# NLESC-JCER/Fortran_Davidson

Hardware: AMD Instinct MI355X
Metric: Davidson iterations/sec (dense DPR solve, matrix resident in HBM) + A*V HBM GB/s vs roofline (higher is better)
Workload: dtype f64

## Files before the change

fortran_davidson_amd/csrc/engine_apply.hip:

```cpp
#include "engine_internal.h"

bool inner_f32_tiles(E* e, OpDesc& o) {
  if (e->inner_bits != 32 || o.kind != DAV_KIND_DENSE || o.storage != 1 || o.a32_refused) return false;
  if (o.a32_valid) return true;
  const size_t count = (size_t)std::max<int64_t>(e->sym.ntiles, 1) * SYM_TB * SYM_TB;
  if (!o.a32 && pool_malloc(&o.a32, sizeof(float) * count) != hipSuccess) {
    (void)hipGetLastError();
    o.a32 = nullptr;
    o.a32_refused = true;
    return false;
  }
  launch_tiles_to_f32(e->stream, o.a, o.a32, (int64_t)count);
  o.a32_valid = true;
  return true;
}

static double* sym_slab_t(const E* e, const SymLaunch& L) { return e->sym_slab + (int64_t)L.ngroups * L.dstride; }
static void sym_sweep(E* e, const SymLaunch& L, const OpDesc& o, const SymSet& set, const double* xt) {
  if (L.nitems == 0) return;
  const SymPlan* pl = L.plan;
  const void* tiles = L.use32 ? (const void*)o.a32 : (const void*)o.a;
  double *slabD = e->sym_slab, *slabT = sym_slab_t(e, L);
  const int64_t xs = e->xt_group_stride, ds = L.dstride, ts = L.tstride;
  switch (L.family) {
    case SYM_ROW_STORED:
      return launch_matvec_sym(e->stream, o.a, set.row_off, set.items, set.nitems, xt, L.kk, slabD, slabT, L.ngroups, xs, ds, ts);
    case SYM_ROW_GENERATED:
      return launch_matvec_sym_generated(e->stream, op_params(o), e->n, set.items, set.nitems, xt, L.kk, slabD, slabT, L.ngroups, xs, ds, ts);
    case SYM_SUPER:
      return launch_matvec_sym9(e->stream, L.R, o.kind != DAV_KIND_DENSE, tiles, L.use32, set.row_off, o.kind != DAV_KIND_DENSE ? op_params(o) : OpParams{},
                                e->n, e->sym_nb, pl->items, pl->nitems, pl->zslot_begin, xt, L.kk, slabD, slabT, L.nwg, xs, ds, ts, e->tune.sym_mfma4 != 0);
    case SYM_WIDE:
    case SYM_WIDE_F32:
      return launch_matvec_symw(e->stream, L.nbw, L.tall, L.use32, tiles, set.row_off, e->sym_nb, pl->items, pl->nitems, pl->zslot_begin, xt, L.kk, slabD, slabT, L.nwg, xs, ds, ts);
    case SYM_WIDE_GENERATED:
      return launch_matvec_symw_generated(e->stream, op_params(o), e->n, e->sym_nb, pl->items, pl->nitems, pl->zslot_begin, xt, L.kk, slabD, slabT, L.nwg, xs, ds, ts);
  }
}

static void count_apply(E* e, int which, int kk) { if (which == DAV_OP_A) { e->st.applies += 1; e->st.apply_cols += kk; } }

static int pack_operand(E* e, const double* src, int kk, bool gather) {
  launch_pack_xt(e->stream, src, e->ldp, e->nloc, e->nslab, kk, e->xt, e->xt_group_stride, e->row0);
  if (!gather) return 0;
  const int ngroups = (kk + 15) / 16;
  CollGroup grp(e);
  CHK(grp.begin(5, 8.0 * (double)e->nslab * 16 * ngroups * e->nranks));
  for (int g = 0; g < ngroups; ++g)
    CHK(coll_allgather(e, e->xt + g * e->xt_group_stride + e->row0 * 16, e->xt + g * e->xt_group_stride, (size_t)e->nslab * 16));
  return grp.end("all-gather of the new block", e->stream);
}

static void sym_reduce_groups(E* e, const SymLaunch& L, const SymSet& set, const int64_t* owned, double* out, int64_t chunk_rows, bool accumulate) {
  const int64_t total_rows = (int64_t)e->nranks * e->nslab;
  const double* slabT = sym_slab_t(e, L);
  for (int g = 0; g < L.ngroups; ++g) {
    const int kg = std::min(16, L.kk - 16 * g);
    const double *d = e->sym_slab + g * L.dstride, *t = slabT + g * L.tstride;
    double* og = out + (size_t)g * 16 * (size_t)(chunk_rows ? total_rows : e->ldp);
    if (L.plan)
      launch_sym9_reduce(e->stream, d, t, L.plan->row_begin, L.plan->zslot_begin, owned, L.plan->next_owned, L.R, e->sym_nb, e->nloc, kg, og, e->ldp,
                         chunk_rows, total_rows, accumulate);
    else
      launch_sym_reduce(e->stream, d, t, set.row_begin, owned, e->sym_nb, e->nloc, kg, og, e->ldp, chunk_rows, total_rows, accumulate);
  }
}

static int ensure_sym_wpart(E* e) {
  if (e->sym_wpart) return 0;
  HIPCHK(pool_malloc(&e->sym_wpart, sizeof(double) * (size_t)e->nranks * (size_t)e->nslab * 64));
  HIPCHK(pool_malloc(&e->sym_wrecv, sizeof(double) * (size_t)e->nslab * 64));
  return 0;
}

static int sym_scatter_to_panel(E* e, int kk, double* dst, bool accumulate, const char* what, double* h0 = nullptr, size_t h0_count = 0) {
  const size_t wstride = (size_t)e->nranks * (size_t)e->nslab * 16, rstride = (size_t)e->nslab * 16;
  const int ngroups = (kk + 15) / 16;
  CollGroup grp(e);
  CHK(grp.begin(6, 8.0 * (double)e->nslab * kk * e->nranks));
  for (int g = 0; g < ngroups; ++g)
    CHK(coll_reduce_scatter(e, e->sym_wpart + g * wstride, e->sym_wrecv + g * rstride, (size_t)e->nslab * std::min(16, kk - 16 * g)));
  if (h0) CHK(coll_allreduce(e, h0, h0_count));
  CHK(grp.end(what, e->stream));
  for (int g = 0; g < ngroups; ++g)
    launch_chunk_to_panel(e->stream, e->sym_wrecv + g * rstride, e->nslab, e->nloc, e->nloc_pad, std::min(16, kk - 16 * g), dst + (int64_t)(16 * g) * e->ldp, e->ldp, accumulate);
  return 0;
}

static double sym_stored_bytes(const E* e, const OpDesc& o, const SymSet& set, bool partial, bool use32) {
  return o.kind != DAV_KIND_DENSE ? 0.0 : (use32 ? 4.0 : 8.0) * (partial ? (double)set.ntiles * SYM_TB * SYM_TB : 0.5 * (double)e->n * ((double)e->n + 1.0) / e->nranks);
}

static int apply_sym_overlapped(E* e, int which, OpDesc& o, const double* src, int k, double* dst, bool timed, bool inner) {
  const int step = 32;
  const int nchunks = (k + step - 1) / step;
  if (!e->ov_ready) {
    hipStream_t cs = nullptr;
    hipEvent_t evs[8] = {};
    double* bufs[4] = {};
    auto undo = [&]() {
      for (hipEvent_t v : evs) if (v) (void)hipEventDestroy(v);
      for (double* b : bufs) if (b) (void)pool_free(b);
      if (cs) (void)hipStreamDestroy(cs);
    };
    int prio_least = 0, prio_greatest = 0;
    if (hipDeviceGetStreamPriorityRange(&prio_least, &prio_greatest) != hipSuccess) { (void)hipGetLastError(); prio_greatest = 0; }
    bool ok = hipStreamCreateWithPriority(&cs, hipStreamNonBlocking, prio_greatest) == hipSuccess;
    for (int i = 0; ok && i < 8; ++i) ok = hipEventCreateWithFlags(&evs[i], hipEventDisableTiming) == hipSuccess;
    for (int i = 0; ok && i < 2; ++i) {
      ok = pool_malloc(&bufs[i], sizeof(double) * (size_t)e->nranks * (size_t)e->nslab * 32) == hipSuccess &&
           pool_malloc(&bufs[2 + i], sizeof(double) * (size_t)e->nslab * 32) == hipSuccess;
    }
    if (!ok) {
      (void)hipGetLastError();
      undo();
      return 2;
    }
    e->comm_stream = cs;
// ... 433 lines not shown
  }
  const bool sym = e->op[which].storage == 1;
  *bytes = (sym ? sym_stored_bytes(e, e->op[which], e->sym, false, false) : 8.0 * (double)e->nloc * (double)e->n) + 16.0 * (double)e->n * k;
  *flops = 2.0 * (sym ? (double)e->n / e->nranks : (double)e->nloc) * (double)e->n * k;
  e->st = saved;
  return 0;
}

extern "C" int dav_bench_stream3(dav_handle_t e, int64_t doubles, int reps, double* copy_GBps, double* triad_GBps, double* read_GBps) {
  CHK(bind(e));
  const int64_t n = doubles > 0 ? doubles / 2 * 2 : (int64_t)1 << 28;
  if (reps <= 0) reps = 5;
  double *a = nullptr, *b = nullptr, *c = nullptr;
  hipEvent_t ev[2] = {nullptr, nullptr};
  auto cleanup = [&]() {
    pool_free(a); pool_free(b); pool_free(c);
    for (hipEvent_t v : ev) if (v) hipEventDestroy(v);
  };
  if (pool_malloc(&a, sizeof(double) * n) != hipSuccess || pool_malloc(&b, sizeof(double) * n) != hipSuccess ||
      pool_malloc(&c, sizeof(double) * n) != hipSuccess || hipEventCreate(&ev[0]) != hipSuccess || hipEventCreate(&ev[1]) != hipSuccess) {
    (void)hipGetLastError();
    cleanup();
    return fail("dav_bench_stream: could not allocate three arrays of " + std::to_string(n) + " doubles");
  }
  double out[3] = {0.0, 0.0, 0.0};
  int rc = 0;
  auto run = [&]() -> int {
    HIPCHK(hipMemsetAsync(b, 0, sizeof(double) * n, e->stream));
    HIPCHK(hipMemsetAsync(c, 0, sizeof(double) * n, e->stream));
    for (int mode = 0; mode < 3; ++mode) {
      launch_stream(e->stream, mode, a, b, c, 0.5, n);
      HIPCHK(hipEventRecord(ev[0], e->stream));
      for (int r = 0; r < reps; ++r) launch_stream(e->stream, mode, a, b, c, 0.5, n);
      HIPCHK(hipEventRecord(ev[1], e->stream));
      HIPCHK(hipEventSynchronize(ev[1]));
      float ms = 0;
      HIPCHK(hipEventElapsedTime(&ms, ev[0], ev[1]));
      out[mode] = (mode == 1 ? 3.0 : 2.0) * 8.0 * (double)n * reps / (ms * 1e-3) / 1e9;
    }
    return 0;
  };
  rc = run();
  cleanup();
  if (rc != 0) return rc;
  if (copy_GBps) *copy_GBps = out[0];
  if (triad_GBps) *triad_GBps = out[1];
  if (read_GBps) *read_GBps = out[2];
  return 0;
}
extern "C" int dav_bench_stream(dav_handle_t e, int64_t doubles, int reps, double* copy_GBps, double* triad_GBps) {
  return dav_bench_stream3(e, doubles, reps, copy_GBps, triad_GBps, nullptr);
}

extern "C" int dav_bench_harness_rate(dav_handle_t e, int iters, double* entries_per_s) {
  CHK(bind(e));
  if (iters <= 0) iters = 2000;
  const int wgs = 512;
  double* out = nullptr;
  hipEvent_t ev[2] = {nullptr, nullptr};
  HIPCHK(pool_malloc(&out, sizeof(double) * (size_t)wgs * 512));
  auto cleanup = [&]() { pool_free(out); for (hipEvent_t v : ev) if (v) hipEventDestroy(v); };
  auto run = [&]() -> int {
    HIPCHK(hipEventCreate(&ev[0]));
    HIPCHK(hipEventCreate(&ev[1]));
    launch_harness_rate(e->stream, out, wgs, 200);
    HIPCHK(hipEventRecord(ev[0], e->stream));
    launch_harness_rate(e->stream, out, wgs, iters);
    HIPCHK(hipEventRecord(ev[1], e->stream));
    HIPCHK(hipEventSynchronize(ev[1]));
    float ms = 0;
    HIPCHK(hipEventElapsedTime(&ms, ev[0], ev[1]));
    *entries_per_s = (double)wgs * 512.0 * iters / (ms * 1e-3);
    return 0;
  };
  const int rc = run();
  cleanup();
  return rc;
}
```

fortran_davidson_amd/csrc/engine_internal.h:

```cpp
#pragma once
#include "davidson_hip_private.h"
#include "kernels.h"
#include "ingest.h"

#include <dlfcn.h>
#include <fcntl.h>
#include <pthread.h>
#include <sys/mman.h>
#include <sys/stat.h>
#include <unistd.h>
#include <rccl/rccl.h>

#include <algorithm>
#include <chrono>
#include <condition_variable>
#include <ctime>
#include <mutex>
#include <cmath>
#include <cstdio>
#include <cstring>
#include <numeric>
#include <string>
#include <thread>
#include <vector>

#pragma GCC visibility push(hidden)
extern thread_local std::string g_err;
int fail(const std::string& msg);
#define HIPCHK(call)                                                                                  \
  do {                                                                                                \
    hipError_t e_ = (call);                                                                           \
    if (e_ != hipSuccess) {                                                                           \
      (void)hipGetLastError();      \
      return fail(std::string(#call) + " failed: " + hipGetErrorString(e_) + " (" __FILE__ ":" +      \
                  std::to_string(__LINE__) + ")");                                                    \
    }                                                                                                 \
  } while (0)
#define CHK(call)            \
  do {                       \
    int r_ = (call);         \
    if (r_ != 0) return r_;  \
  } while (0)

hipError_t pool_malloc_raw(void** p, size_t bytes);
hipError_t pool_host_malloc_raw(void** p, size_t bytes, unsigned flags);
hipError_t pool_free(void* p);
hipError_t pool_host_free(void* p);
size_t pool_idle_device_bytes(int device);
void pool_begin_of_destroy();
void pool_end_of_destroy();
hipError_t pool_stream_get(hipStream_t* st);
void pool_stream_put(hipStream_t st, int device);
template <class T> inline hipError_t pool_malloc(T** p, size_t bytes) { return pool_malloc_raw((void**)p, bytes); }
template <class T> inline hipError_t pool_host_malloc(T** p, size_t bytes, unsigned flags) { return pool_host_malloc_raw((void**)p, bytes, flags); }


struct Rccl {
  void* lib = nullptr;
  ncclResult_t (*GetUniqueId)(ncclUniqueId*) = nullptr;
  ncclResult_t (*CommInitRank)(ncclComm_t*, int, ncclUniqueId, int) = nullptr;
  ncclResult_t (*CommDestroy)(ncclComm_t) = nullptr;
  ncclResult_t (*AllGather)(const void*, void*, size_t, ncclDataType_t, ncclComm_t, hipStream_t) = nullptr;
  ncclResult_t (*AllReduce)(const void*, void*, size_t, ncclDataType_t, ncclRedOp_t, ncclComm_t, hipStream_t) = nullptr;
  ncclResult_t (*Broadcast)(const void*, void*, size_t, ncclDataType_t, int, ncclComm_t, hipStream_t) = nullptr;
  ncclResult_t (*ReduceScatter)(const void*, void*, size_t, ncclDataType_t, ncclRedOp_t, ncclComm_t, hipStream_t) = nullptr;
  ncclResult_t (*Send)(const void*, size_t, ncclDataType_t, int, ncclComm_t, hipStream_t) = nullptr;
  ncclResult_t (*Recv)(void*, size_t, ncclDataType_t, int, ncclComm_t, hipStream_t) = nullptr;
  ncclResult_t (*GroupStart)() = nullptr;
  ncclResult_t (*GroupEnd)() = nullptr;
  const char* (*GetErrorString)(ncclResult_t) = nullptr;
  ncclResult_t (*CommCount)(const ncclComm_t, int*) = nullptr;
};
extern Rccl g_rccl;
int rccl_load();
#define NCCLCHK(call)                                                                              \
  do {                                                                                             \
    ncclResult_t r_ = (call);                                                                      \
// ... 350 lines not shown
```

fortran_davidson_amd/csrc/k_matvec_sym.hip:

```cpp
#include "kernels.h"
#include <cstdlib>
#include <type_traits>

__device__ __forceinline__ const double* sym_tile(const double* tiles, const int64_t* __restrict__ row_off, int I, int J) {
  return tiles + (row_off[I] + J) * (int64_t)(SYM_TB * SYM_TB);
}

constexpr int SYM8_DEPTH = 3;

template <bool GEN>
__global__ __launch_bounds__(512, 1) void matvec_sym8_kernel(const double* __restrict__ tiles, const int64_t* __restrict__ row_off,
                                                             const int* __restrict__ items,
                                                             const double* __restrict__ xt, double* __restrict__ slabD,
                                                             double* __restrict__ slabT, int kcols, int npair,
                                                             int64_t xt_gstride, int64_t slabD_gstride, int64_t slabT_gstride,
                                                             OpParams op, int64_t n) {
  int item, grp;
  if (npair == 2) {
    const int nfull = (int)(gridDim.x / 16) * 16;
    if ((int)blockIdx.x < nfull) {
      item = (blockIdx.x / 16) * 8 + (blockIdx.x % 8);
      grp = (blockIdx.x / 8) % 2;
    } else {
      item = nfull / 2 + (blockIdx.x - nfull) / 2;
// ... 163 lines not shown
#pragma unroll
          for (int reg = 0; reg < 4; ++reg) zs[4 * reg] = z[reg];
        }
      }
      if ((q & 3) == 3 && ((q >> 2) + 1) % zslots == 0) {
        __syncthreads();
        flush_tiles((q >> 2) + 1 - zslots, zslots);
        __syncthreads();
      }
    }
#pragma unroll
    for (int u = 0; u < 4; ++u) b[u] = bn[u];
  };
  int q = 0;
  for (; q < nq_off; ++q) unit(std::true_type{}, q);
  if ((nq_off >> 2) % zslots != 0) {
    __syncthreads();
    flush_tiles((nq_off >> 2) - (nq_off >> 2) % zslots, (nq_off >> 2) % zslots);
  }
  for (; q < nunits; ++q) unit(std::false_type{}, q);

  double* outD = slabD + (int64_t)items[4 * item + 3] * 16 * SYM_TB;
#pragma unroll
  for (int hs = 0; hs < 4; ++hs) {
    __syncthreads();
#pragma unroll
    for (int par = 0; par < 2; ++par)
#pragma unroll
      for (int reg = 0; reg < 4; ++reg) tw[c * RS + 2 * (g + 4 * reg) + par] = acc[hs][par][reg];
    __syncthreads();
#pragma unroll
    for (int t = 0; t < 2; ++t) {
      const int e = threadIdx.x + 512 * t;
      const int hh = e >> 9, bc = (e >> 5) & 15, r = e & 31;
      const double* rp = tr + (hh * 4) * TRW + bc * RS + r;
      if (bc < kcols) outD[(int64_t)bc * SYM_TB + 128 * hh + 32 * hs + r] = (rp[0] + rp[TRW]) + (rp[2 * TRW] + rp[3 * TRW]);
    }
  }
}

void launch_matvec_sym(hipStream_t st, const double* tiles, const int64_t* row_off, const int* items_dev, int nitems, const double* xt, int kcols,
                       double* slabD, double* slabT, int npair, int64_t xt_gstride, int64_t slabD_gstride, int64_t slabT_gstride) {
  hipLaunchKernelGGL(matvec_sym8_kernel<false>, dim3(nitems * npair), dim3(512), 0, st, tiles, row_off, items_dev, xt, slabD, slabT, kcols,
                     npair, xt_gstride, slabD_gstride, slabT_gstride, OpParams{}, (int64_t)0);
}
void launch_matvec_sym_generated(hipStream_t st, OpParams op, int64_t n, const int* items_dev, int nitems, const double* xt, int kcols,
                                 double* slabD, double* slabT, int npair, int64_t xt_gstride, int64_t slabD_gstride,
                                 int64_t slabT_gstride) {
  hipLaunchKernelGGL(matvec_sym8_kernel<true>, dim3(nitems * npair), dim3(512), 0, st, (const double*)nullptr, (const int64_t*)nullptr, items_dev, xt, slabD,
                     slabT, kcols, npair, xt_gstride, slabD_gstride, slabT_gstride, op, n);
}

__global__ __launch_bounds__(256) void sym_reduce_kernel(const double* __restrict__ slabD, const double* __restrict__ slabT,
                                                         const int* __restrict__ row_item_begin, const int64_t* __restrict__ owned,
                                                         int nb, int ncol16, int64_t nloc, int k, double* __restrict__ dst, int64_t ldd,
                                                         int64_t chunk_rows, int64_t total_rows, int accumulate) {
  const int J = blockIdx.x, col = blockIdx.y, r = threadIdx.x;
  if (col >= k) return;
  double sum = 0.0;
  for (int it = row_item_begin[J]; it < row_item_begin[J + 1]; ++it)
    sum += slabD[((int64_t)it * ncol16 + col) * SYM_TB + r];
  auto zt = [&](int I) { return (!owned || owned[I] >= 0) ? slabT[((((int64_t)I * (I - 1) / 2 + J) * ncol16) + col) * SYM_TB + r] : 0.0; };
  double s0 = 0.0, s1 = 0.0, s2 = 0.0, s3 = 0.0;
  int I = J + 1;
  for (; I + 3 < nb; I += 4) { s0 += zt(I); s1 += zt(I + 1); s2 += zt(I + 2); s3 += zt(I + 3); }
  for (; I < nb; ++I) s0 += zt(I);
  sum += (s0 + s1) + (s2 + s3);
  int64_t row = (int64_t)J * SYM_TB + r;
  if (chunk_rows > 0) {
    if (row < total_rows) dst[(row / chunk_rows) * (chunk_rows * k) + (int64_t)col * chunk_rows + row % chunk_rows] = sum;
  } else {
    dst[(int64_t)col * ldd + row] = row < nloc ? (accumulate ? dst[(int64_t)col * ldd + row] + sum : sum) : 0.0;
  }
}

void launch_sym_reduce(hipStream_t st, const double* slabD, const double* slabT, const int* row_item_begin_dev, const int64_t* owned,
                       int nb, int64_t nloc, int k, double* dst, int64_t ldd, int64_t chunk_rows, int64_t total_rows, bool accumulate) {
  hipLaunchKernelGGL(sym_reduce_kernel, dim3(nb, k), dim3(256), 0, st, slabD, slabT, row_item_begin_dev, owned, nb, 16, nloc, k,
                     dst, ldd, chunk_rows, total_rows, accumulate && chunk_rows == 0 ? 1 : 0);
}

__global__ __launch_bounds__(256) void generate_sym_tiles_kernel(double* __restrict__ row_tiles, int I, int64_t n, uint64_t seed,
                                                                 double sparsity, int use_diag, double diag_val) {
  const int64_t J = blockIdx.x;
  double* tile = row_tiles + J * (int64_t)(SYM_TB * SYM_TB);
  int64_t gi = (int64_t)I * SYM_TB + threadIdx.x;
  for (int cc = 0; cc < 16; ++cc) {
    int64_t lc = blockIdx.y * 16 + cc, gj = J * SYM_TB + lc;
    double v = 0.0;
    if (gi < n && gj < n) v = dav_hashed_entry(seed, sparsity, use_diag, diag_val, gi, gj);
    tile[lc * SYM_TB + threadIdx.x] = v;
  }
}

void launch_generate_sym_tiles(hipStream_t st, double* tiles, const int64_t* row_off_host, int nb, int64_t n, uint64_t seed,
                               double sparsity, int use_diag, double diag_val) {
  for (int I = 0; I < nb; ++I)
    if (row_off_host[I] >= 0)
      hipLaunchKernelGGL(generate_sym_tiles_kernel, dim3((unsigned)(I + 1), SYM_TB / 16), dim3(SYM_TB), 0, st,
                         tiles + row_off_host[I] * (int64_t)(SYM_TB * SYM_TB), I, n, seed, sparsity, use_diag, diag_val);
}

__device__ __forceinline__ double sym_entry(const double* tiles, const int64_t* __restrict__ row_off, int64_t i, int64_t j) {
  if (i < j) { int64_t t = i; i = j; j = t; }
  int I = (int)(i / SYM_TB), J = (int)(j / SYM_TB);
  if (row_off[I] < 0) return 0.0;
  return sym_tile(tiles, row_off, I, J)[(j % SYM_TB) * SYM_TB + (i % SYM_TB)];
}

__global__ void diag_sym_kernel(const double* __restrict__ tiles, const int64_t* __restrict__ row_off, int64_t n, int64_t nrows,
                                double* __restrict__ diag) {
  int64_t i = (int64_t)blockIdx.x * 256 + threadIdx.x;
  if (i < nrows) diag[i] = i < n ? sym_entry(tiles, row_off, i, i) : 0.0;
}
void launch_diag_sym(hipStream_t st, const double* tiles, const int64_t* row_off, int64_t n, int64_t nrows, double* diag) {
  hipLaunchKernelGGL(diag_sym_kernel, dim3((unsigned)((nrows + 255) / 256)), dim3(256), 0, st, tiles, row_off, n, nrows, diag);
}

__global__ void gather_columns_sym_kernel(const double* __restrict__ tiles, const int64_t* __restrict__ row_off, int64_t n,
                                          int64_t nrows_pad, const int64_t* __restrict__ idx, double* __restrict__ dst, int64_t ldd) {
  int64_t i = (int64_t)blockIdx.x * 256 + threadIdx.x;
  int c = blockIdx.y;
  if (i < nrows_pad) dst[(int64_t)c * ldd + i] = i < n ? sym_entry(tiles, row_off, i, idx[c]) : 0.0;
}
void launch_gather_columns_sym(hipStream_t st, const double* tiles, const int64_t* row_off, int64_t n, int64_t nrows_pad,
                               const int64_t* idx_dev, int k, double* dst, int64_t ldd) {
  hipLaunchKernelGGL(gather_columns_sym_kernel, dim3((unsigned)((nrows_pad + 255) / 256), k), dim3(256), 0, st, tiles, row_off, n,
                     nrows_pad, idx_dev, dst, ldd);
}

__global__ void gather_columns_sym_rs_kernel(const double* __restrict__ tiles, const int64_t* __restrict__ row_off, int64_t n,
// ... 36 lines not shown
```

fortran_davidson_amd/csrc/k_matvec_sym9.hip:

```cpp
#include "kernels.h"
#include <cstdlib>
#include <type_traits>

__device__ __forceinline__ const double* sym9_tile(const double* tiles, const int64_t* __restrict__ row_off, int I, int J) {
  return tiles + (row_off[I] + J) * (int64_t)(SYM_TB * SYM_TB);
}

__device__ __forceinline__ double mfma4_f64(double a, double b, double c) { return __builtin_amdgcn_mfma_f64_4x4x4f64(a, b, c, 0, 0, 0); }

template <int R, bool GEN, bool F32, bool M4, int HARN = 0>
__global__ __launch_bounds__(512, 1) void matvec_sym9_kernel(const void* __restrict__ tiles_v, const int64_t* __restrict__ row_off,
                                                             const int* __restrict__ items,
                                                             const int* __restrict__ zslot_begin, const double* __restrict__ xt,
                                                             double* __restrict__ slabD, double* __restrict__ slabT, int kcols,
                                                             int npair, int64_t xt_gstride, int64_t slabD_gstride,
                                                             int64_t slabT_gstride, int nb, OpParams op, int64_t n) {
  const double* tiles = static_cast<const double*>(tiles_v);
  const float* tiles32 = static_cast<const float*>(tiles_v);
  (void)tiles; (void)tiles32;
  constexpr int NCG = 4 / R;
  constexpr int NRS = 2 * R;
  constexpr int BW = 16 * NCG;
  constexpr int UPJ = SYM_TB / BW;
  constexpr int UPS = 64 / BW;
// ... 305 lines not shown
#pragma unroll
    for (int t = 0; t < NRS; ++t) {
      const int e = threadIdx.x + 512 * t;
      const int sl = e >> 9, bc = (e >> 5) & 15, r = e & 31;
      const double* rp = tr + (sl * NCG) * TRW + bc * RS + r;
      double sum = rp[0];
#pragma unroll
      for (int ww = 1; ww < NCG; ++ww) sum += rp[ww * TRW];
      if (bc < kcols) outD[((int64_t)(sl >> 1) * 16 + bc) * SYM_TB + 128 * (sl & 1) + 32 * hs + r] = sum;
    }
  }
}

void launch_matvec_sym9(hipStream_t st, int R, bool gen, const void* tiles, bool tiles_f32, const int64_t* row_off, OpParams op, int64_t n,
                        int nb, const int* items_dev, int nitems, const int* zslot_begin_dev, const double* xt, int kcols, double* slabD,
                        double* slabT, int npair, int64_t xt_gstride, int64_t slabD_gstride, int64_t slabT_gstride, bool m4) {
  dim3 grid(nitems * npair), block(512);
#define DAV_SYM9_LAUNCH(RR, GG, FF, MM, ...)                                                                                     \
  hipLaunchKernelGGL((matvec_sym9_kernel<RR, GG, FF, MM, ##__VA_ARGS__>), grid, block, 0, st, tiles, row_off, items_dev, zslot_begin_dev, xt, slabD, slabT, \
                     kcols, npair, xt_gstride, slabD_gstride, slabT_gstride, nb, op, n)
  const bool harness = gen && op.kind == DAV_KIND_HARNESS;
  const bool hsin = harness && op.trig != 0;
  const bool hlibm = harness && op.libm != 0;
  if (R == 4) {
    if (hlibm) DAV_SYM9_LAUNCH(4, true, false, true, 3);
    else if (hsin) DAV_SYM9_LAUNCH(4, true, false, true, 2);
    else if (harness) DAV_SYM9_LAUNCH(4, true, false, true, 1);
    else if (gen) DAV_SYM9_LAUNCH(4, true, false, true);
    else if (tiles_f32) DAV_SYM9_LAUNCH(4, false, true, true);
    else if (m4) DAV_SYM9_LAUNCH(4, false, false, true);
    else DAV_SYM9_LAUNCH(4, false, false, false);
  } else {
    if (hlibm) DAV_SYM9_LAUNCH(2, true, false, false, 3);
    else if (hsin) DAV_SYM9_LAUNCH(2, true, false, false, 2);
    else if (harness) DAV_SYM9_LAUNCH(2, true, false, false, 1);
    else if (gen) DAV_SYM9_LAUNCH(2, true, false, false);
    else if (tiles_f32) DAV_SYM9_LAUNCH(2, false, true, false);
    else DAV_SYM9_LAUNCH(2, false, false, false);
  }
#undef DAV_SYM9_LAUNCH
}

__global__ __launch_bounds__(256) void tiles_to_f32_kernel(const double* __restrict__ src, float* __restrict__ dst, int64_t count4) {
  for (int64_t e = (int64_t)blockIdx.x * 256 + threadIdx.x; e < count4; e += (int64_t)gridDim.x * 256) {
    const f64x2 a = reinterpret_cast<const f64x2*>(src)[2 * e], b = reinterpret_cast<const f64x2*>(src)[2 * e + 1];
    reinterpret_cast<float4*>(dst)[e] = float4{(float)a.x, (float)a.y, (float)b.x, (float)b.y};
  }
}
void launch_tiles_to_f32(hipStream_t st, const double* src, float* dst, int64_t count) {
  hipLaunchKernelGGL(tiles_to_f32_kernel, dim3(256 * 32), dim3(256), 0, st, src, dst, count / 4);
}

__global__ __launch_bounds__(256) void sym9_reduce_kernel(const double* __restrict__ slabD, const double* __restrict__ slabT,
                                                          const int* __restrict__ row_item_begin, const int* __restrict__ zslot_begin,
                                                          const int64_t* __restrict__ owned, const int* __restrict__ next_owned, int R, int nb,
                                                          int nsuper, int64_t nloc, int k, double* __restrict__ dst, int64_t ldd,
                                                          int64_t chunk_rows, int64_t total_rows, int accumulate) {
  const int J = blockIdx.x, col = blockIdx.y, r = threadIdx.x;
  if (col >= k) return;
  double sum = 0.0;
  const int Sown = J / R, sub = J % R;
  for (int it = row_item_begin[Sown]; it < row_item_begin[Sown + 1]; ++it)
    sum += slabD[(((int64_t)it * R + sub) * 16 + col) * SYM_TB + r];
  auto zt = [&](int S) { return slabT[(((int64_t)zslot_begin[S] + J) * 16 + col) * SYM_TB + r]; };
  double s0 = 0.0, s1 = 0.0, s2 = 0.0, s3 = 0.0;
  const int Send = (nb - 1 > J) ? nsuper : 0;
  if (!owned) {
    int S = (J + 1) / R;
    for (; S + 3 < Send; S += 4) { s0 += zt(S); s1 += zt(S + 1); s2 += zt(S + 2); s3 += zt(S + 3); }
    for (; S < Send; ++S) s0 += zt(S);
  } else {
    int S = (J + 1) / R < nsuper ? next_owned[(J + 1) / R] : nsuper;
    while (S < Send) {
      s0 += zt(S); S = next_owned[S + 1];
      if (S >= Send) break;
      s1 += zt(S); S = next_owned[S + 1];
      if (S >= Send) break;
      s2 += zt(S); S = next_owned[S + 1];
      if (S >= Send) break;
      s3 += zt(S); S = next_owned[S + 1];
    }
  }
  sum += (s0 + s1) + (s2 + s3);
  const int64_t row = (int64_t)J * SYM_TB + r;
  if (chunk_rows > 0) {
    if (row < total_rows) dst[(row / chunk_rows) * (chunk_rows * k) + (int64_t)col * chunk_rows + row % chunk_rows] = sum;
  } else {
    dst[(int64_t)col * ldd + row] = row < nloc ? (accumulate ? dst[(int64_t)col * ldd + row] + sum : sum) : 0.0;
  }
}

void launch_sym9_reduce(hipStream_t st, const double* slabD, const double* slabT, const int* row_item_begin_dev,
                        const int* zslot_begin_dev, const int64_t* owned, const int* next_owned, int R, int nb, int64_t nloc, int k, double* dst,
                        int64_t ldd, int64_t chunk_rows, int64_t total_rows, bool accumulate) {
  const int nsuper = (nb + R - 1) / R;
  hipLaunchKernelGGL(sym9_reduce_kernel, dim3(nb, k), dim3(256), 0, st, slabD, slabT, row_item_begin_dev, zslot_begin_dev, owned, next_owned, R,
                     nb, nsuper, nloc, k, dst, ldd, chunk_rows, total_rows, accumulate && chunk_rows == 0 ? 1 : 0);
}
```

fortran_davidson_amd/csrc/kernels.h:

```cpp
#pragma once
#include "common.h"

constexpr int MV_ROWS = 256;
void launch_pack_xt(hipStream_t st, const double* src, int64_t ld, int64_t nloc, int64_t nslab, int k,
                    double* xt, int64_t xt_group_stride, int64_t row_off);
void launch_matvec_dense(hipStream_t st, const double* A, int64_t lda, int64_t nrows_pad, int64_t ncols_pad,
                         const double* xt, int64_t xt_group_stride, int ngroups, double* slab,
                         int nsplit, int jc);
void launch_matvec_free(hipStream_t st, OpParams op, int64_t row0, int64_t nloc, int64_t n,
                        int64_t nrows_pad, int64_t ncols_pad, const double* xt, int64_t xt_group_stride,
                        int ngroups, double* slab, int nsplit, int jc);
void launch_slab_reduce(hipStream_t st, const double* slab, int nsplit, int64_t nrows_pad, int ngroups,
                        int64_t nloc, int k, double* dst, int64_t ldd);
size_t matvec_slab_doubles(int64_t nrows_pad, int ngroups, int nsplit);
void matvec_plan(int64_t nrows_pad, int64_t ncols_pad, int ngroups, int* nsplit, int* jc, int64_t target = 0, int64_t forced_nsplit = 0);

constexpr int GRAM_MIN_ROWS = 256;
constexpr int GRAM_FUSE_CHUNKS = 24;
constexpr int GRAM_MAX_COUNTERS = 256;
void launch_gram(hipStream_t st, const double* P, int64_t ldp, int p, const double* Q, int64_t ldq, int q,
                 int64_t nrows_pad, double* scratch, double* out_dev, unsigned* counters = nullptr, int wg_target = 0);
size_t gram_scratch_doubles(int p, int q, int64_t nrows_pad);
void gram_set_fuse_chunks(int n);
void launch_gram_multi(hipStream_t st, const double* P, int64_t ldp, int p, const double* const* Qs, int nq, int qeach, int64_t ldq,
// ... 12 lines not shown
  int batch; int64_t batch_stride;
};
static inline int64_t pg_image_tiles(int q) { return ((int64_t)(q > 0 ? q : 1) + 63) / 64 * 4; }
static inline int64_t pg_image_doubles(int p, int q) { return ((int64_t)(p > 0 ? p : 1) + 3) / 4 * pg_image_tiles(q) * 64; }
static inline int64_t pg_image_index(int i, int j, int64_t tp) { return (((int64_t)(i >> 2) * tp + (j >> 4)) << 6) + (j & 15) + 16 * (i & 3); }
constexpr int PG_ROWS = 128;
constexpr int PG_FUSE_BLOCKS = 48;
constexpr int PG_INPLACE_COLS = 64;
void launch_panel_gemm(hipStream_t st, const PanelGemmArgs& a);
void launch_norm_finish(hipStream_t st, const double* partial, int nblocks, int nnorm, double* out);

void launch_generate_dense(hipStream_t st, double* A, int64_t lda, int64_t nrows_pad, int64_t ncols_pad,
                           int64_t row0, int64_t nloc, int64_t n, uint64_t seed, double sparsity,
                           int use_diag, double diag_val);
void launch_diag_dense(hipStream_t st, const double* A, int64_t lda, int64_t row0, int64_t nloc, double* diag);
void launch_diag_free(hipStream_t st, OpParams op, int64_t row0, int64_t nloc, double* diag);
void launch_gather_columns(hipStream_t st, const double* A, int64_t lda, int64_t nrows_pad,
                           const int64_t* idx_dev, int k, double* dst, int64_t ldd);
void launch_unit_columns(hipStream_t st, const int64_t* idx_dev, int k, int64_t row0, int64_t nloc,
                         int64_t nrows_pad, double* dst, int64_t ldd);
void launch_copy_columns(hipStream_t st, const double* src, int64_t lds, double* dst, int64_t ldd,
                         int64_t nrows_pad, int k);
void launch_stream(hipStream_t st, int mode, double* a, const double* b, const double* c, double s, int64_t n);
void launch_harness_rate(hipStream_t st, double* out, int wgs, int iters);
void launch_compare_blocks(hipStream_t st, const double* a, const double* b, int64_t ld, int64_t rows, int k, double* out);
void launch_poke(hipStream_t st, double* p, double delta);
void launch_sum_parts(hipStream_t st, const double* own, const double* stage, int nparts, int self, size_t count, double* out);



void launch_rows_scatter(hipStream_t st, const double* stage, int64_t ldr, int64_t grow0, int64_t nrows, int64_t n,
                         double* dst, int64_t lda, int64_t slab_row0, int64_t slab_rows, int sym, const int64_t* row_off);

struct LincombArgs {
  const double* in[4]; const double* coef; int ldc; int nterms;
  double* out; int64_t ld; int64_t nrows_pad; int m;
};
void launch_lincomb(hipStream_t st, const LincombArgs& a);
void launch_precond(hipStream_t st, const double* in, double* out, int64_t ld, int64_t nloc, int64_t nrows_pad, int m,
                    const double* theta, const double* dA, const double* dB, const double* active);
struct DotsArgs {
  const double* a[4]; const double* b[4]; int npairs; int64_t ld; int64_t nrows_pad; int m; double* partial;
};
int coldots_blocks(int64_t nrows_pad);
void launch_coldots(hipStream_t st, const DotsArgs& a);

constexpr int SYM_TB = 256;
void launch_matvec_sym(hipStream_t st, const double* tiles, const int64_t* row_off, const int* items_dev, int nitems, const double* xt, int kcols,
                       double* slabD, double* slabT, int npair, int64_t xt_gstride, int64_t slabD_gstride, int64_t slabT_gstride);
void launch_matvec_sym_generated(hipStream_t st, OpParams op, int64_t n, const int* items_dev, int nitems, const double* xt, int kcols,
                                 double* slabD, double* slabT, int npair, int64_t xt_gstride, int64_t slabD_gstride,
                                 int64_t slabT_gstride);
void launch_sym_reduce(hipStream_t st, const double* slabD, const double* slabT, const int* row_item_begin_dev, const int64_t* owned,
                       int nb, int64_t nloc, int k, double* dst, int64_t ldd, int64_t chunk_rows, int64_t total_rows, bool accumulate = false);
void launch_matvec_sym9(hipStream_t st, int R, bool gen, const void* tiles, bool tiles_f32, const int64_t* row_off, OpParams op, int64_t n,
                        int nb, const int* items_dev, int nitems, const int* zslot_begin_dev, const double* xt, int kcols, double* slabD,
                        double* slabT, int npair, int64_t xt_gstride, int64_t slabD_gstride, int64_t slabT_gstride, bool mfma4 = true);
void launch_matvec_symw(hipStream_t st, int nbw, bool tall, bool tiles_f32, const void* tiles, const int64_t* row_off, int nb, const int* items_dev,
                        int nitems, const int* zslot_begin_dev, const double* xt, int kcols, double* slabD, double* slabT, int nwg,
                        int64_t xt_gstride, int64_t slabD_gstride, int64_t slabT_gstride);
void launch_matvec_symw_generated(hipStream_t st, OpParams op, int64_t n, int nb, const int* items_dev, int nitems, const int* zslot_begin_dev,
                                  const double* xt, int kcols, double* slabD, double* slabT, int nwg, int64_t xt_gstride, int64_t slabD_gstride,
                                  int64_t slabT_gstride);
void launch_tiles_to_f32(hipStream_t st, const double* src, float* dst, int64_t count);
void launch_sym9_reduce(hipStream_t st, const double* slabD, const double* slabT, const int* row_item_begin_dev,
                        const int* zslot_begin_dev, const int64_t* owned, const int* next_owned, int R, int nb, int64_t nloc, int k, double* dst,
                        int64_t ldd, int64_t chunk_rows, int64_t total_rows, bool accumulate = false);
void launch_generate_sym_tiles(hipStream_t st, double* tiles, const int64_t* row_off_host, int nb, int64_t n, uint64_t seed,
                               double sparsity, int use_diag, double diag_val);
void launch_retile_panel(hipStream_t st, const double* panel, int64_t ldp, int64_t nrows, int ncols, int J, int nb,
                         const int64_t* row_off, double* tiles);
void launch_diag_sym(hipStream_t st, const double* tiles, const int64_t* row_off, int64_t n, int64_t nrows, double* diag);
void launch_gather_columns_sym_rs(hipStream_t st, const double* tiles, const int64_t* row_off, int64_t n, int64_t chunk_rows,
                                  int64_t total_rows, const int64_t* idx_dev, int k, double* dst);
void launch_entries_sym(hipStream_t st, const double* tiles, const int64_t* row_off, const int64_t* idx_dev, int k, double* h0);
void launch_zero_pad_rows(hipStream_t st, double* dst, int64_t ldd, int64_t nloc, int64_t nrows_pad, int k);
void launch_entries_free(hipStream_t st, OpParams op, const int64_t* idx_dev, int k, double* h0);
void launch_entries_dense(hipStream_t st, const double* A, int64_t lda, const int64_t* idx_dev, int k, double* h0);
void launch_gather_columns_free(hipStream_t st, OpParams op, int64_t row0, int64_t nloc, int64_t nrows_pad, const int64_t* idx_dev, int k,
                                double* dst, int64_t ldd);
void launch_gather_columns_sym(hipStream_t st, const double* tiles, const int64_t* row_off, int64_t n, int64_t nrows_pad,
                               const int64_t* idx_dev, int k, double* dst, int64_t ldd);
void launch_chunk_to_panel(hipStream_t st, const double* src, int64_t lds, int64_t nloc, int64_t nrows_pad, int k, double* dst, int64_t ldd,
                           bool accumulate = false);

constexpr int CSR_ROWS = 16;
constexpr int64_t CSR_CHUNK = 1024;
struct CsrItem { int64_t p0, p1; int32_t row, nrows, slot, pad; };
struct CsrLong { int32_t row, first, count, pad; };
void launch_spmm_csr(hipStream_t st, const CsrItem* items, int nitems, const int64_t* rp, const int32_t* col, const double* val,
                     const double* xt, int64_t xt_gstride, int groups, int kk, double* part, double* dst, int64_t ldd);
void launch_spmm_csr_finish(hipStream_t st, const CsrLong* longs, int nlong, const double* part, int kk, double* dst, int64_t ldd);
struct ChebEpi { const double *z, *r, *zprev, *hdr, *ab, *pi; int64_t ld; };
void launch_spmm_csr_cheb(hipStream_t st, const CsrItem* items, int nitems, const int64_t* rp, const int32_t* col, const double* val,
                          const double* xt, int64_t xt_gstride, int groups, int kk, double* part, double* dst, int64_t ldd, const ChebEpi& epi);
void launch_spmm_csr_finish_cheb(hipStream_t st, const CsrLong* longs, int nlong, const double* part, int kk, double* dst, int64_t ldd,
                                 const ChebEpi& epi);

template <class F> void cb_dispatch(int rp64, int ci64, F&& f) {
  if (rp64) {
    if (ci64) f(int64_t{}, int64_t{});
    else f(int64_t{}, int32_t{});
  } else {
    if (ci64) f(int32_t{}, int64_t{});
    else f(int32_t{}, int32_t{});
  }
}

void launch_csr_build_rows(hipStream_t st, const void* rp, int rp64, int64_t n, unsigned long long* info);
void launch_csr_build_check(hipStream_t st, const void* rp, int rp64, const void* col, int ci64, int64_t n, int64_t nnz, int base, int lower,
                            int64_t r0, int64_t nloc, unsigned long long* first_bad, int32_t* mcount, uint32_t* dcount,
                            unsigned long long* dfirst);
void launch_csr_build_locate(hipStream_t st, const void* rp, int rp64, const void* col, int ci64, int64_t n, int base, int64_t p, int64_t* out);
void launch_csr_build_offsets(hipStream_t st, const void* rp, int rp64, int64_t r0, int64_t nloc, const int32_t* mcount, int64_t* lrp,
                              int64_t* tile_sums);
int64_t csr_build_scan_tiles(int64_t m);
void launch_csr_build_scan(hipStream_t st, int64_t* x, int64_t m, int64_t* tile_sums);
void launch_csr_build_scatter(hipStream_t st, const void* rp, int rp64, const void* col, int ci64, const double* vals, int64_t n, int64_t p_lo,
                              int64_t p_hi, int base, int lower, int64_t r0, int64_t nloc, const int64_t* lrp, int32_t* fill, int32_t* ocol,
                              double* oval, uint32_t* tie);
// ... 73 lines not shown
```

Before: 22.78.

## Fuse per-group symmetric reduce launches into one vectorized multi-column kernel

Replaces the per-16-column-group loop of sym/sym9 reduce launches with a single launch covering all groups. Each block now handles a column pair with f64x2 row loads, and the transpose-candidate sum is compacted through a shared-memory offset list built with wave ballots, then streamed with four accumulators. This is meant to cut launch count and the scalar, strided reads of the reduction phase. The summation order changes, so a new order-check test entry point compares the result against the old kernels, kept as reference versions.

```diff
diff --git a/fortran_davidson_amd/csrc/engine_apply.hip b/fortran_davidson_amd/csrc/engine_apply.hip
--- a/fortran_davidson_amd/csrc/engine_apply.hip
+++ b/fortran_davidson_amd/csrc/engine_apply.hip
@@ -54,16 +54,13 @@
 static void sym_reduce_groups(E* e, const SymLaunch& L, const SymSet& set, const int64_t* owned, double* out, int64_t chunk_rows, bool accumulate) {
   const int64_t total_rows = (int64_t)e->nranks * e->nslab;
   const double* slabT = sym_slab_t(e, L);
-  for (int g = 0; g < L.ngroups; ++g) {
-    const int kg = std::min(16, L.kk - 16 * g);
-    const double *d = e->sym_slab + g * L.dstride, *t = slabT + g * L.tstride;
-    double* og = out + (size_t)g * 16 * (size_t)(chunk_rows ? total_rows : e->ldp);
-    if (L.plan)
-      launch_sym9_reduce(e->stream, d, t, L.plan->row_begin, L.plan->zslot_begin, owned, L.plan->next_owned, L.R, e->sym_nb, e->nloc, kg, og, e->ldp,
-                         chunk_rows, total_rows, accumulate);
-    else
-      launch_sym_reduce(e->stream, d, t, set.row_begin, owned, e->sym_nb, e->nloc, kg, og, e->ldp, chunk_rows, total_rows, accumulate);
-  }
+  const int64_t ostride = 16 * (chunk_rows ? total_rows : e->ldp);
+  if (L.plan)
+    launch_sym9_reduce(e->stream, e->sym_slab, slabT, L.plan->row_begin, L.plan->zslot_begin, owned, L.plan->next_owned, L.R, e->sym_nb, e->nloc, L.kk,
+                       L.ngroups, L.dstride, L.tstride, out, ostride, e->ldp, chunk_rows, total_rows, accumulate);
+  else
+    launch_sym_reduce(e->stream, e->sym_slab, slabT, set.row_begin, owned, e->sym_nb, e->nloc, L.kk, L.ngroups, L.dstride, L.tstride, out, ostride,
+                      e->ldp, chunk_rows, total_rows, accumulate);
 }
 
 static int ensure_sym_wpart(E* e) {
@@ -603,6 +600,83 @@
   return dav_bench_stream3(e, doubles, reps, copy_GBps, triad_GBps, nullptr);
 }
 
+extern "C" int symtest_reduce_order_check(dav_handle_t e, int R, int kk, uint64_t seed, int chunked, int accumulate, int64_t* words_compared,
+                                          int64_t* words_different, int64_t* sentinels_lost) {
+  CHK(bind(e));
+  if (e->storage != 1) return fail("symtest_reduce_order_check: the engine is not in symmetric-tiled storage mode (dav_set_storage)");
+  if ((R != 1 && R != 2 && R != 4) || kk < 1 || kk > 64 || (R == 4 && kk > 16)) return fail("symtest_reduce_order_check: R in {1, 2, 4}, kk in 1..64, R = 4 up to 16 columns");
+  if (e->nranks > 1 && !chunked) return fail("symtest_reduce_order_check: a rank of several sums into the reduce-scatter layout only");
+  if (chunked && accumulate) return fail("symtest_reduce_order_check: the reduce-scatter layout is never accumulated into");
+  CHK(sym_setup(e));
+  const SymSet& set = e->sym;
+  OpDesc stored;
+  stored.kind = DAV_KIND_DENSE;
+  const SymLaunch L = sym_launch(e, stored, set, kk, false, R);
+  const int64_t nrows = (int64_t)e->sym_nb * SYM_TB, total_rows = (int64_t)e->nranks * e->nslab;
+  if (!chunked && e->ldp < nrows) return fail("symtest_reduce_order_check: panel columns shorter than the block rows");
+  CHK(sym_ensure_slabs(e, (size_t)L.ngroups * (size_t)(L.dstride + L.tstride) + 1));
+  const int64_t chunk_rows = chunked ? e->nslab : 0;
+  const int64_t* owned = (e->nranks > 1 || chunked) ? set.row_off : nullptr;
+  const int64_t guard = 512, gstride = 16 * (chunked ? total_rows : e->ldp), span = L.ngroups * gstride, words = span + 2 * guard;
+  const uint64_t sentinel = 0x7FF8C0DEC0DEC0DEull;
+  double* buf[2] = {nullptr, nullptr};
+  auto cleanup = [&]() { pool_free(buf[0]); pool_free(buf[1]); };
+  std::vector<uint64_t> start((size_t)words, sentinel), host[2];
+  auto run = [&]() -> int {
+    for (double*& b : buf) HIPCHK(pool_malloc(&b, sizeof(double) * (size_t)words));
+    launch_sym_order_fill(e->stream, e->sym_slab, L.ngroups * (L.dstride + L.tstride), seed);
+    if (accumulate) {
+      launch_sym_order_fill(e->stream, buf[0], words, seed + 1);
+      HIPCHK(hipMemcpyAsync(start.data(), buf[0], sizeof(double) * (size_t)words, hipMemcpyDeviceToHost, e->stream));
+      HIPCHK(hipMemcpyAsync(buf[1], buf[0], sizeof(double) * (size_t)words, hipMemcpyDeviceToDevice, e->stream));
+    } else {
+      for (double* b : buf) HIPCHK(hipMemcpyAsync(b, start.data(), sizeof(double) * (size_t)words, hipMemcpyHostToDevice, e->stream));
+    }
+    const double* slabT = sym_slab_t(e, L);
+    for (int g = 0; g < L.ngroups; ++g) {
+      const int kg = std::min(16, kk - 16 * g);
+      const double *d = e->sym_slab + g * L.dstride, *t = slabT + g * L.tstride;
+      double* og = buf[0] + guard + g * gstride;
+      if (L.plan)
+        launch_sym9_reduce_order_reference(e->stream, d, t, L.plan->row_begin, L.plan->zslot_begin, owned, L.plan->next_owned, L.R, e->sym_nb, e->nloc, kg,
+                                           og, e->ldp, chunk_rows, total_rows, accumulate != 0);
+      else
+        launch_sym_reduce_order_reference(e->stream, d, t, set.row_begin, owned, e->sym_nb, e->nloc, kg, og, e->ldp, chunk_rows, total_rows, accumulate != 0);
+    }
+    sym_reduce_groups(e, L, set, owned, buf[1] + guard, chunk_rows, accumulate != 0);
+    HIPCHK(hipGetLastError());
+    for (int b = 0; b < 2; ++b) {
+      host[b].resize((size_t)words);
+      HIPCHK(hipMemcpyAsync(host[b].data(), buf[b], sizeof(double) * (size_t)words, hipMemcpyDeviceToHost, e->stream));
+    }
+    HIPCHK(hipStreamSynchronize(e->stream));
+    return 0;
+  };
+  const int rc = run();
+  if (rc != 0) (void)hipStreamSynchronize(e->stream);
+  cleanup();
+  if (rc != 0) return rc;
+  std::vector<char> written((size_t)words, 0);
+  for (int g = 0; g < L.ngroups; ++g) {
+    const int kg = std::min(16, kk - 16 * g);
+    for (int c = 0; c < kg; ++c)
+      for (int64_t row = 0; row < nrows; ++row) {
+        if (chunked && row >= total_rows) break;
+        const int64_t at = chunked ? (row / chunk_rows) * (chunk_rows * kg) + c * chunk_rows + row % chunk_rows : c * e->ldp + row;
+        written[(size_t)(guard + g * gstride + at)] = 1;
+      }
+  }
+  int64_t differ = 0, lost = 0;
+  for (int64_t i = 0; i < words; ++i) {
+    if (host[0][(size_t)i] != host[1][(size_t)i]) ++differ;
+    if (!written[(size_t)i] && host[1][(size_t)i] != start[(size_t)i]) ++lost;
+  }
+  if (words_compared) *words_compared = words;
+  if (words_different) *words_different = differ;
+  if (sentinels_lost) *sentinels_lost = lost;
+  return 0;
+}
+
 extern "C" int dav_bench_harness_rate(dav_handle_t e, int iters, double* entries_per_s) {
   CHK(bind(e));
   if (iters <= 0) iters = 2000;
diff --git a/fortran_davidson_amd/csrc/engine_internal.h b/fortran_davidson_amd/csrc/engine_internal.h
--- a/fortran_davidson_amd/csrc/engine_internal.h
+++ b/fortran_davidson_amd/csrc/engine_internal.h
@@ -23,6 +23,9 @@
 #include <string>
 #include <thread>
 #include <vector>
+
+extern "C" int symtest_reduce_order_check(dav_handle_t h, int R, int kk, uint64_t seed, int chunked, int accumulate, int64_t* words_compared,
+                                          int64_t* words_different, int64_t* sentinels_lost);
 
 #pragma GCC visibility push(hidden)
 extern thread_local std::string g_err;
diff --git a/fortran_davidson_amd/csrc/k_matvec_sym.hip b/fortran_davidson_amd/csrc/k_matvec_sym.hip
--- a/fortran_davidson_amd/csrc/k_matvec_sym.hip
+++ b/fortran_davidson_amd/csrc/k_matvec_sym.hip
@@ -239,6 +239,50 @@
 }
 
 __global__ __launch_bounds__(256) void sym_reduce_kernel(const double* __restrict__ slabD, const double* __restrict__ slabT,
+                                                         const int* __restrict__ row_item_begin, const int64_t* __restrict__ owned,
+                                                         int nb, int ncol16, int64_t nloc, int kk, int64_t dstride, int64_t tstride,
+                                                         double* __restrict__ dst, int64_t ostride, int64_t ldd, int64_t chunk_rows,
+                                                         int64_t total_rows, int accumulate) {
+  __shared__ SymRedList list;
+  const int J = blockIdx.y, grp = blockIdx.x >> 3, pair = blockIdx.x & 7, t = threadIdx.x;
+  const int k = kk - 16 * grp < 16 ? kk - 16 * grp : 16;
+  if (2 * pair >= k) return;
+  const int col = 2 * pair + (t >> 7), r2 = 2 * (t & 127);
+  const int64_t slot = (int64_t)ncol16 * SYM_TB;
+  f64x2 sum = f64x2{0.0, 0.0};
+  {
+    const double* pd = slabD + grp * dstride + col * SYM_TB + r2;
+    auto dt = [&](int it) { return *reinterpret_cast<const f64x2*>(pd + (int64_t)it * slot); };
+    int it = row_item_begin[J];
+    const int it1 = row_item_begin[J + 1];
+    for (; it + 8 <= it1; it += 8) {
+      f64x2 v[8];
+#pragma unroll
+      for (int u = 0; u < 8; ++u) v[u] = dt(it + u);
+#pragma unroll
+      for (int u = 0; u < 8; ++u) sum += v[u];
+    }
+    for (; it < it1; ++it) sum += dt(it);
+  }
+  f64x2 s[4] = {f64x2{0.0, 0.0}, f64x2{0.0, 0.0}, f64x2{0.0, 0.0}, f64x2{0.0, 0.0}};
+  const double* pt = slabT + grp * tstride + (int64_t)J * slot + col * SYM_TB + r2;
+  symred_sum_candidates<true>(list, pt, J + 1, nb, true,
+                              [&](int I, int64_t* off) {
+                                *off = (!owned || owned[I] >= 0) ? (int64_t)I * (I - 1) / 2 * slot : (int64_t)-1;
+                                return true;
+                              }, s);
+  sum += (s[0] + s[1]) + (s[2] + s[3]);
+  if (col < k) symred_store(dst + grp * ostride, sum, (int64_t)J * SYM_TB + r2, col, k, nloc, ldd, chunk_rows, total_rows, accumulate);
+}
+
+void launch_sym_reduce(hipStream_t st, const double* slabD, const double* slabT, const int* row_item_begin_dev, const int64_t* owned,
+                       int nb, int64_t nloc, int kk, int ngroups, int64_t dstride, int64_t tstride, double* dst, int64_t ostride, int64_t ldd,
+                       int64_t chunk_rows, int64_t total_rows, bool accumulate) {
+  hipLaunchKernelGGL(sym_reduce_kernel, dim3(8 * ngroups, nb), dim3(256), 0, st, slabD, slabT, row_item_begin_dev, owned, nb, 16, nloc, kk,
+                     dstride, tstride, dst, ostride, ldd, chunk_rows, total_rows, accumulate && chunk_rows == 0 ? 1 : 0);
+}
+
+__global__ __launch_bounds__(256) void sym_reduce_order_reference_kernel(const double* __restrict__ slabD, const double* __restrict__ slabT,
                                                          const int* __restrict__ row_item_begin, const int64_t* __restrict__ owned,
                                                          int nb, int ncol16, int64_t nloc, int k, double* __restrict__ dst, int64_t ldd,
                                                          int64_t chunk_rows, int64_t total_rows, int accumulate) {
@@ -261,9 +305,9 @@
   }
 }
 
-void launch_sym_reduce(hipStream_t st, const double* slabD, const double* slabT, const int* row_item_begin_dev, const int64_t* owned,
-                       int nb, int64_t nloc, int k, double* dst, int64_t ldd, int64_t chunk_rows, int64_t total_rows, bool accumulate) {
-  hipLaunchKernelGGL(sym_reduce_kernel, dim3(nb, k), dim3(256), 0, st, slabD, slabT, row_item_begin_dev, owned, nb, 16, nloc, k,
+void launch_sym_reduce_order_reference(hipStream_t st, const double* slabD, const double* slabT, const int* row_item_begin_dev, const int64_t* owned,
+                                       int nb, int64_t nloc, int k, double* dst, int64_t ldd, int64_t chunk_rows, int64_t total_rows, bool accumulate) {
+  hipLaunchKernelGGL(sym_reduce_order_reference_kernel, dim3(nb, k), dim3(256), 0, st, slabD, slabT, row_item_begin_dev, owned, nb, 16, nloc, k,
                      dst, ldd, chunk_rows, total_rows, accumulate && chunk_rows == 0 ? 1 : 0);
 }
 
diff --git a/fortran_davidson_amd/csrc/k_matvec_sym9.hip b/fortran_davidson_amd/csrc/k_matvec_sym9.hip
--- a/fortran_davidson_amd/csrc/k_matvec_sym9.hip
+++ b/fortran_davidson_amd/csrc/k_matvec_sym9.hip
@@ -381,6 +381,57 @@
 }
 
 __global__ __launch_bounds__(256) void sym9_reduce_kernel(const double* __restrict__ slabD, const double* __restrict__ slabT,
+                                                          const int* __restrict__ row_item_begin, const int* __restrict__ zslot_begin,
+                                                          const int64_t* __restrict__ owned, const int* __restrict__ next_owned, int R, int nb,
+                                                          int nsuper, int64_t nloc, int kk, int64_t dstride, int64_t tstride,
+                                                          double* __restrict__ dst, int64_t ostride, int64_t ldd, int64_t chunk_rows,
+                                                          int64_t total_rows, int accumulate) {
+  __shared__ SymRedList list;
+  const int J = blockIdx.y, grp = blockIdx.x >> 3, pair = blockIdx.x & 7, t = threadIdx.x;
+  const int k = kk - 16 * grp < 16 ? kk - 16 * grp : 16;
+  if (2 * pair >= k) return;
+  const int col = 2 * pair + (t >> 7), r2 = 2 * (t & 127);
+  constexpr int64_t SLOT = 16 * SYM_TB;
+  const int Sown = J / R, sub = J % R;
+  f64x2 sum = f64x2{0.0, 0.0};
+  {
+    const double* pd = slabD + grp * dstride + (int64_t)sub * SLOT + col * SYM_TB + r2;
+    auto dt = [&](int it) { return *reinterpret_cast<const f64x2*>(pd + (int64_t)it * R * SLOT); };
+    int it = row_item_begin[Sown];
+    const int it1 = row_item_begin[Sown + 1];
+    for (; it + 8 <= it1; it += 8) {
+      f64x2 v[8];
+#pragma unroll
+      for (int u = 0; u < 8; ++u) v[u] = dt(it + u);
+#pragma unroll
+      for (int u = 0; u < 8; ++u) sum += v[u];
+    }
+    for (; it < it1; ++it) sum += dt(it);
+  }
+  f64x2 s[4] = {f64x2{0.0, 0.0}, f64x2{0.0, 0.0}, f64x2{0.0, 0.0}, f64x2{0.0, 0.0}};
+  const int Send = (nb - 1 > J) ? nsuper : 0;
+  const double* pt = slabT + grp * tstride + (int64_t)J * SLOT + col * SYM_TB + r2;
+  if (!owned)
+    symred_sum_candidates<false>(list, pt, (J + 1) / R, Send, true,
+                                 [&](int S, int64_t* off) { *off = (int64_t)zslot_begin[S] * SLOT; return true; }, s);
+  else
+    symred_sum_candidates<false>(list, pt, (J + 1) / R, Send, false,
+                                 [&](int S, int64_t* off) { *off = (int64_t)zslot_begin[S] * SLOT; return next_owned[S] == S; }, s);
+  sum += (s[0] + s[1]) + (s[2] + s[3]);
+  if (col < k) symred_store(dst + grp * ostride, sum, (int64_t)J * SYM_TB + r2, col, k, nloc, ldd, chunk_rows, total_rows, accumulate);
+}
+
+void launch_sym9_reduce(hipStream_t st, const double* slabD, const double* slabT, const int* row_item_begin_dev,
+                        const int* zslot_begin_dev, const int64_t* owned, const int* next_owned, int R, int nb, int64_t nloc, int kk, int ngroups,
+                        int64_t dstride, int64_t tstride, double* dst, int64_t ostride, int64_t ldd, int64_t chunk_rows, int64_t total_rows,
+                        bool accumulate) {
+  const int nsuper = (nb + R - 1) / R;
+  hipLaunchKernelGGL(sym9_reduce_kernel, dim3(8 * ngroups, nb), dim3(256), 0, st, slabD, slabT, row_item_begin_dev, zslot_begin_dev, owned,
+                     next_owned, R, nb, nsuper, nloc, kk, dstride, tstride, dst, ostride, ldd, chunk_rows, total_rows,
+                     accumulate && chunk_rows == 0 ? 1 : 0);
+}
+
+__global__ __launch_bounds__(256) void sym9_reduce_order_reference_kernel(const double* __restrict__ slabD, const double* __restrict__ slabT,
                                                           const int* __restrict__ row_item_begin, const int* __restrict__ zslot_begin,
                                                           const int64_t* __restrict__ owned, const int* __restrict__ next_owned, int R, int nb,
                                                           int nsuper, int64_t nloc, int k, double* __restrict__ dst, int64_t ldd,
@@ -419,10 +470,23 @@
   }
 }
 
-void launch_sym9_reduce(hipStream_t st, const double* slabD, const double* slabT, const int* row_item_begin_dev,
-                        const int* zslot_begin_dev, const int64_t* owned, const int* next_owned, int R, int nb, int64_t nloc, int k, double* dst,
-                        int64_t ldd, int64_t chunk_rows, int64_t total_rows, bool accumulate) {
+void launch_sym9_reduce_order_reference(hipStream_t st, const double* slabD, const double* slabT, const int* row_item_begin_dev,
+                                        const int* zslot_begin_dev, const int64_t* owned, const int* next_owned, int R, int nb, int64_t nloc, int k,
+                                        double* dst, int64_t ldd, int64_t chunk_rows, int64_t total_rows, bool accumulate) {
   const int nsuper = (nb + R - 1) / R;
-  hipLaunchKernelGGL(sym9_reduce_kernel, dim3(nb, k), dim3(256), 0, st, slabD, slabT, row_item_begin_dev, zslot_begin_dev, owned, next_owned, R,
-                     nb, nsuper, nloc, k, dst, ldd, chunk_rows, total_rows, accumulate && chunk_rows == 0 ? 1 : 0);
-}
+  hipLaunchKernelGGL(sym9_reduce_order_reference_kernel, dim3(nb, k), dim3(256), 0, st, slabD, slabT, row_item_begin_dev, zslot_begin_dev, owned,
+                     next_owned, R, nb, nsuper, nloc, k, dst, ldd, chunk_rows, total_rows, accumulate && chunk_rows == 0 ? 1 : 0);
+}
+
+__global__ __launch_bounds__(256) void sym_order_fill_kernel(double* __restrict__ p, int64_t count, uint64_t seed) {
+  for (int64_t i = (int64_t)blockIdx.x * 256 + threadIdx.x; i < count; i += (int64_t)gridDim.x * 256) {
+    const uint64_t h = dav_splitmix64(seed * 0x9E3779B97F4A7C15ull + (uint64_t)i);
+    const uint64_t expo = 1023 - 30 + (h >> 52) % 61;
+    p[i] = __longlong_as_double((long long)((h << 63) | (expo << 52) | ((h >> 1) & 0x000FFFFFFFFFFFFFull)));
+  }
+}
+void launch_sym_order_fill(hipStream_t st, double* p, int64_t count, uint64_t seed) {
+  if (count <= 0) return;
+  const int64_t blocks = (count + 255) / 256;
+  hipLaunchKernelGGL(sym_order_fill_kernel, dim3((unsigned)(blocks < 4096 ? blocks : 4096)), dim3(256), 0, st, p, count, seed);
+}
diff --git a/fortran_davidson_amd/csrc/kernels.h b/fortran_davidson_amd/csrc/kernels.h
--- a/fortran_davidson_amd/csrc/kernels.h
+++ b/fortran_davidson_amd/csrc/kernels.h
@@ -88,7 +88,8 @@
                                  double* slabD, double* slabT, int npair, int64_t xt_gstride, int64_t slabD_gstride,
                                  int64_t slabT_gstride);
 void launch_sym_reduce(hipStream_t st, const double* slabD, const double* slabT, const int* row_item_begin_dev, const int64_t* owned,
-                       int nb, int64_t nloc, int k, double* dst, int64_t ldd, int64_t chunk_rows, int64_t total_rows, bool accumulate = false);
+                       int nb, int64_t nloc, int kk, int ngroups, int64_t dstride, int64_t tstride, double* dst, int64_t ostride, int64_t ldd,
+                       int64_t chunk_rows, int64_t total_rows, bool accumulate = false);
 void launch_matvec_sym9(hipStream_t st, int R, bool gen, const void* tiles, bool tiles_f32, const int64_t* row_off, OpParams op, int64_t n,
                         int nb, const int* items_dev, int nitems, const int* zslot_begin_dev, const double* xt, int kcols, double* slabD,
                         double* slabT, int npair, int64_t xt_gstride, int64_t slabD_gstride, int64_t slabT_gstride, bool mfma4 = true);
@@ -100,8 +101,104 @@
                                   int64_t slabT_gstride);
 void launch_tiles_to_f32(hipStream_t st, const double* src, float* dst, int64_t count);
 void launch_sym9_reduce(hipStream_t st, const double* slabD, const double* slabT, const int* row_item_begin_dev,
-                        const int* zslot_begin_dev, const int64_t* owned, const int* next_owned, int R, int nb, int64_t nloc, int k, double* dst,
-                        int64_t ldd, int64_t chunk_rows, int64_t total_rows, bool accumulate = false);
+                        const int* zslot_begin_dev, const int64_t* owned, const int* next_owned, int R, int nb, int64_t nloc, int kk, int ngroups,
+                        int64_t dstride, int64_t tstride, double* dst, int64_t ostride, int64_t ldd, int64_t chunk_rows, int64_t total_rows,
+                        bool accumulate = false);
+void launch_sym_reduce_order_reference(hipStream_t st, const double* slabD, const double* slabT, const int* row_item_begin_dev, const int64_t* owned,
+                                       int nb, int64_t nloc, int k, double* dst, int64_t ldd, int64_t chunk_rows, int64_t total_rows, bool accumulate);
+void launch_sym9_reduce_order_reference(hipStream_t st, const double* slabD, const double* slabT, const int* row_item_begin_dev,
+                                        const int* zslot_begin_dev, const int64_t* owned, const int* next_owned, int R, int nb, int64_t nloc, int k,
+                                        double* dst, int64_t ldd, int64_t chunk_rows, int64_t total_rows, bool accumulate);
+void launch_sym_order_fill(hipStream_t st, double* p, int64_t count, uint64_t seed);
+
+constexpr int SYMRED_WINDOW = 256;
+constexpr int SYMRED_CAP = 4 * SYMRED_WINDOW;
+struct SymRedList {
+  int64_t offs[SYMRED_CAP];
+  int wave_count[4];
+};
+template <bool ZERO_TERMS>
+__device__ __forceinline__ void symred_stream(const double* __restrict__ p, const int64_t* offs, int n, bool tail_s0, f64x2 (&s)[4]) {
+  auto term = [&](int i) -> f64x2 {
+    const int64_t o = offs[i];
+    if constexpr (ZERO_TERMS) {
+      if (o < 0) return f64x2{0.0, 0.0};
+    }
+    return *reinterpret_cast<const f64x2*>(p + o);
+  };
+  const int n4 = n & ~3;
+  int i = 0;
+  for (; i + 8 <= n4; i += 8) {
+    f64x2 v[8];
+#pragma unroll
+    for (int u = 0; u < 8; ++u) v[u] = term(i + u);
+#pragma unroll
+    for (int u = 0; u < 8; ++u) s[u & 3] += v[u];
+  }
+  if (i < n4) {
+    f64x2 v[4];
+#pragma unroll
+    for (int u = 0; u < 4; ++u) v[u] = term(i + u);
+#pragma unroll
+    for (int u = 0; u < 4; ++u) s[u] += v[u];
+    i += 4;
+  }
+  f64x2 v[3];
+#pragma unroll
+  for (int u = 0; u < 3; ++u) v[u] = i + u < n ? term(i + u) : f64x2{0.0, 0.0};
+#pragma unroll
+  for (int u = 0; u < 3; ++u)
+    if (i + u < n) {
+      if (tail_s0) s[0] += v[u];
+      else s[u] += v[u];
+    }
+}
+template <bool ZERO_TERMS, class F>
+__device__ __forceinline__ void symred_sum_candidates(SymRedList& L, const double* __restrict__ p, int c0, int c1, bool tail_s0, F&& offset_of,
+                                                      f64x2 (&s)[4]) {
+  const int t = threadIdx.x, lane = t & 63, wave = t >> 6;
+  int cnt = 0;
+  for (int w0 = c0; w0 < c1; w0 += SYMRED_WINDOW) {
+    const int c = w0 + t;
+    int64_t off = -1;
+    const bool take = c < c1 && offset_of(c, &off);
+    const unsigned long long mask = __ballot(take);
+    if (lane == 0) L.wave_count[wave] = __popcll(mask);
+    __syncthreads();
+    int before = cnt, total = 0;
+#pragma unroll
+    for (int w = 0; w < 4; ++w) {
+      const int wc = L.wave_count[w];
+      if (w < wave) before += wc;
+      total += wc;
+    }
+    if (take) L.offs[before + __popcll(mask & ((1ull << lane) - 1ull))] = off;
+    cnt += total;
+    __syncthreads();
+    const bool last = w0 + SYMRED_WINDOW >= c1;
+    if (last || cnt > SYMRED_CAP - SYMRED_WINDOW) {
+      const int n = last ? cnt : cnt & ~7;
+      symred_stream<ZERO_TERMS>(p, L.offs, n, last && tail_s0, s);
+      const int left = cnt - n;
+      const int64_t keep = t < left ? L.offs[n + t] : 0;
+      __syncthreads();
+      if (t < left) L.offs[t] = keep;
+      cnt = left;
+    }
+  }
+}
+__device__ __forceinline__ void symred_store(double* __restrict__ dst, f64x2 sum, int64_t row, int col, int k, int64_t nloc, int64_t ldd,
+                                             int64_t chunk_rows, int64_t total_rows, int accumulate) {
+#pragma unroll
+  for (int h = 0; h < 2; ++h, ++row) {
+    const double v = h == 0 ? sum.x : sum.y;
+    if (chunk_rows > 0) {
+      if (row < total_rows) dst[(row / chunk_rows) * (chunk_rows * k) + (int64_t)col * chunk_rows + row % chunk_rows] = v;
+    } else {
+      dst[(int64_t)col * ldd + row] = row < nloc ? (accumulate ? dst[(int64_t)col * ldd + row] + v : v) : 0.0;
+    }
+  }
+}
 void launch_generate_sym_tiles(hipStream_t st, double* tiles, const int64_t* row_off_host, int nb, int64_t n, uint64_t seed,
                                double sparsity, int use_diag, double diag_val);
 void launch_retile_panel(hipStream_t st, const double* panel, int64_t ldp, int64_t nrows, int ncols, int J, int nb,
```

Result: no change. 22.83, median of 6 (+0.2%).
